# facebookresearch/vilbert-multi-task

Hardware: AMD Instinct MI355X
Metric: samples/sec (36 regions, 36 tokens) ViLBERT-base 6L/6C fwd+bwd (higher is better)
Workload: dtype f32; 1 GPU; bert_base_6layer_6conect.json train_concap step: BertForMultiModalPreTraining fwd+bwd (dropout on) + grad all-reduce + AdamW, 36 regions + 1 global row, batch 256 per GPU, T=36 R=37; per_gpu_batch=256, global_batch=256, parallelism=dp1, visible_gpus=1, launch=eager, gemm_mode=f32, deterministic_wgrad=True, deterministic_fallbacks=0

## Files before the change

### vilbert-multi-task_amd/csrc/attention.hip

```cpp
#include "common.h"
#include "rng.h"

namespace {

#ifdef VB_ATTN_BF16
typedef unsigned short io_t;
__device__ __forceinline__ f32x4 ld4(const io_t* p) {
    const uint2 w = *reinterpret_cast<const uint2*>(p);
    return f32x4{__uint_as_float(w.x << 16), __uint_as_float(w.x & 0xffff0000u), __uint_as_float(w.y << 16),
                 __uint_as_float(w.y & 0xffff0000u)};
}
__device__ __forceinline__ float ld1(const io_t* p) { return __uint_as_float((unsigned)*p << 16); }
__device__ __forceinline__ void st1(io_t* p, float v) { *p = (io_t)vb_bf16_round(v); }
template <int DS>
__device__ __forceinline__ void store_cols(io_t* op, int c, const f32x4 (&a)[DS], int r) {
#pragma unroll
    for (int k = 0; k < DS / 2; ++k) {
        const float even = a[2 * k][r], odd = a[2 * k + 1][r];
        const float recv = __shfl_xor((c & 1) ? even : odd, 1, 64);
        if (c & 1) *reinterpret_cast<unsigned*>(op + 32 * k + 15) = vb_bf16_pack(recv, odd);
        else *reinterpret_cast<unsigned*>(op + 32 * k) = vb_bf16_pack(even, recv);
    }
}
#else
// ... 212 lines not shown
#pragma unroll
                for (int r = 0; r < 4; ++r) st[kt][r] = st[kt][r] * (dp[kt][r] - dsum) * p.scale;
    }

    const io_t* rbase = (BWD ? kbase : vbase) + c;
    const long ldr = BWD ? p.ldk : p.ldv;
    f32x4 oacc[DS];
#pragma unroll
    for (int dt = 0; dt < DS; ++dt) oacc[dt] = f32x4{0.f, 0.f, 0.f, 0.f};
#pragma unroll
    for (int kt = 0; kt < NT; ++kt) {
        if (kt < nkt) {
            f32x4 av, bv[DS];
#pragma unroll
            for (int r = 0; r < 4; ++r) {
                const int key = min(kt * 16 + 4 * g + r, p.n_k - 1);
                const io_t* rp = rbase + (long)key * ldr;
                av[r] = st[kt][r];
#pragma unroll
                for (int dt = 0; dt < DS; ++dt) bv[dt][r] = ld1(rp + 16 * dt);
            }
            mma_rank4<DS>(oacc, av, bv);
        }
    }

    io_t* obase = BWD ? p.dQ : p.O;
    const long ldo = BWD ? p.lddq : p.ldo;
#pragma unroll
    for (int r = 0; r < 4; ++r) {
        const int q = qt * 16 + 4 * g + r;
        if (q < p.n_q) {
            io_t* op = obase + ((long)b * p.n_q + q) * ldo + h * D + c;
            store_cols<DS>(op, c, oacc, r);
        }
    }
}

template <int D>
__global__ __launch_bounds__(256) void attn_bwd_kv_kernel(const AttnP p_in) {
    AttnP p = p_in;
    p.seed = vb_seed_with_epoch(p_in.seed, p_in.epoch);
    const int lane = threadIdx.x & 63;
    const long item = (long)blockIdx.x * 4 + (threadIdx.x >> 6);
    if (item >= p.total) return;
    const int kt = (int)(item % p.n_kt);
    const long bh = item / p.n_kt;
    const int h = (int)(bh % p.heads);
    const int b = (int)(bh / p.heads);
    const int c = lane & 15, g = lane >> 4;
    constexpr int DS = D / 16;
    const bool drop = p.drop_p > 0.f;

    const int key = kt * 16 + c;
    const int k_row = min(key, p.n_k - 1);
    const bool key_ok = key < p.n_k;
    f32x4 kf[DS], vf[DS];
    load_frag<DS>(kf, p.K + ((long)b * p.n_k + k_row) * p.ldk + h * D + 4 * g);
    load_frag<DS>(vf, p.V + ((long)b * p.n_k + k_row) * p.ldv + h * D + 4 * g);
    const float madd = p.mask != nullptr ? p.mask[(long)b * p.n_k + k_row] : 0.f;

    const io_t* qbase = p.Q + (long)b * p.n_q * p.ldq + h * D;
    const io_t* dobase = p.dO + (long)b * p.n_q * p.lddo + h * D;
    const float* lse = p.lse + bh * p.n_q;
    const float* dvec = p.dvec + bh * p.n_q;

    f32x4 dk[DS], dv[DS];
#pragma unroll
    for (int dt = 0; dt < DS; ++dt) {
        dk[dt] = f32x4{0.f, 0.f, 0.f, 0.f};
        dv[dt] = f32x4{0.f, 0.f, 0.f, 0.f};
    }

    for (int qt = 0; qt < p.n_qt; ++qt) {
        const int q_row = min(qt * 16 + c, p.n_q - 1);
        f32x4 qf[DS], dof[DS];
        load_frag<DS>(qf, qbase + (long)q_row * p.ldq + 4 * g);
        load_frag<DS>(dof, dobase + (long)q_row * p.lddo + 4 * g);
        const f32x4 s = dot_tile<DS>(qf, kf);
        const f32x4 dpr = dot_tile<DS>(dof, vf);
        f32x4 pd, dsv;
#pragma unroll
        for (int r = 0; r < 4; ++r) {
            const int q = qt * 16 + 4 * g + r;
            float dsr = 0.f, pdr = 0.f;
            if (q < p.n_q && key_ok) {
                const float sv = __fadd_rn(__fmul_rn(s[r], p.scale), madd);
                const float pv = expf(sv - lse[q]);
                float d = dpr[r];
                pdr = pv;
                if (drop) {
                    const bool keep = vb_keep(p.seed, (uint64_t)((bh * p.n_q + q) * p.n_k + key), p.drop_p);
                    d = keep ? d * p.drop_scale : 0.f;
                    pdr = keep ? pv * p.drop_scale : 0.f;
                }
                dsr = pv * (d - dvec[q]) * p.scale;
            }
            pd[r] = pdr;
            dsv[r] = dsr;
        }
        f32x4 dov[DS], qv[DS];
#pragma unroll
        for (int r = 0; r < 4; ++r) {
            const int q = min(qt * 16 + 4 * g + r, p.n_q - 1);
            const io_t* dop = dobase + (long)q * p.lddo + c;
            const io_t* qp = qbase + (long)q * p.ldq + c;
#pragma unroll
            for (int dt = 0; dt < DS; ++dt) {
                dov[dt][r] = ld1(dop + 16 * dt);
                qv[dt][r] = ld1(qp + 16 * dt);
            }
        }
        mma_rank4<DS>(dv, pd, dov);
        mma_rank4<DS>(dk, dsv, qv);
    }

#pragma unroll
    for (int r = 0; r < 4; ++r) {
        const int kk = kt * 16 + 4 * g + r;
        if (kk < p.n_k) {
            io_t* kp = p.dK + ((long)b * p.n_k + kk) * p.lddk + h * D + c;
            io_t* vp = p.dV + ((long)b * p.n_k + kk) * p.lddv + h * D + c;
            store_cols<DS>(kp, c, dk, r);
            store_cols<DS>(vp, c, dv, r);
        }
    }
}

constexpr int LDS_MAX_ROWS = 48;

template <int D>
__device__ __forceinline__ void stage_rows2(float* __restrict__ s0, const io_t* __restrict__ g0, long ld0,
                                            float* __restrict__ s1, const io_t* __restrict__ g1, long ld1, int n_rows) {
    constexpr int V4 = D / 4, IT = (LDS_MAX_ROWS * V4 + 255) / 256;
    f32x4 r0[IT], r1[IT];
#pragma unroll
    for (int i = 0; i < IT; ++i) {
        const int f = threadIdx.x + 256 * i;
        const int r = min(f / V4, n_rows - 1), c4 = f % V4;
        r0[i] = ld4(g0 + (long)r * ld0 + c4 * 4);
        r1[i] = ld4(g1 + (long)r * ld1 + c4 * 4);
    }
#pragma unroll
    for (int i = 0; i < IT; ++i) {
        const int f = threadIdx.x + 256 * i;
        const int r = f / V4, c4 = f % V4;
        if (f < LDS_MAX_ROWS * V4) {
            const bool real = r < n_rows;
            *reinterpret_cast<f32x4*>(s0 + r * (D + 4) + c4 * 4) = real ? r0[i] : f32x4{0.f, 0.f, 0.f, 0.f};
            *reinterpret_cast<f32x4*>(s1 + r * (D + 4) + c4 * 4) = real ? r1[i] : f32x4{0.f, 0.f, 0.f, 0.f};
        }
    }
}

template <int DS>
__device__ __forceinline__ void load_frag_lds(f32x4 (&f)[DS], const float* s) {
#pragma unroll
    for (int q = 0; q < DS; ++q) f[q] = *reinterpret_cast<const f32x4*>(s + 16 * q);
}

template <int D, bool BWD>
__global__ __launch_bounds__(256, 3) void attn_q_lds_kernel(const AttnP p_in) {
    AttnP p = p_in;
    p.seed = vb_seed_with_epoch(p_in.seed, p_in.epoch);
    extern __shared__ __attribute__((aligned(16))) float smem_att[];
    constexpr int LD = D + 4, DS = D / 16, NT = LDS_MAX_ROWS / 16;
    float* sK = smem_att;
    float* sV = smem_att + LDS_MAX_ROWS * LD;
    const long bh = blockIdx.x;
    const int h = (int)(bh % p.heads), b = (int)(bh / p.heads);
    const int lane = threadIdx.x & 63, wave = threadIdx.x >> 6;
    const int c = lane & 15, g = lane >> 4;
    const int nkt = p.n_kt;
    const bool drop = p.drop_p > 0.f;

    f32x4 qf_first[DS];
    load_frag<DS>(qf_first, p.Q + ((long)b * p.n_q + min(wave * 16 + c, p.n_q - 1)) * p.ldq + h * D + 4 * g);
    stage_rows2<D>(sK, p.K + (long)b * p.n_k * p.ldk + h * D, p.ldk, sV, p.V + (long)b * p.n_k * p.ldv + h * D, p.ldv, p.n_k);
    __syncthreads();
    const float* mrow = p.mask != nullptr ? p.mask + (long)b * p.n_k : nullptr;

    for (int qt = wave; qt < p.n_qt; qt += 4) {
        const int q_row = min(qt * 16 + c, p.n_q - 1);
        f32x4 qf[DS];
        if (qt == wave) {
#pragma unroll
            for (int i = 0; i < DS; ++i) qf[i] = qf_first[i];
        } else {
            load_frag<DS>(qf, p.Q + ((long)b * p.n_q + q_row) * p.ldq + h * D + 4 * g);
        }
        const long prow = (bh * p.n_q + q_row) * p.n_k;

        f32x4 st[NT];
        float mx = -INFINITY;
#pragma unroll
        for (int kt = 0; kt < NT; ++kt) {
            st[kt] = f32x4{-INFINITY, -INFINITY, -INFINITY, -INFINITY};
            if (kt < nkt) {
                f32x4 kf[DS];
                load_frag_lds<DS>(kf, sK + (kt * 16 + c) * LD + 4 * g);
                f32x4 acc = dot_tile<DS>(kf, qf);
#pragma unroll
                for (int r = 0; r < 4; ++r) {
                    const int key = kt * 16 + 4 * g + r;
                    float v = -INFINITY;
                    if (key < p.n_k) {
                        v = __fmul_rn(acc[r], p.scale);
                        if (mrow != nullptr) v = __fadd_rn(v, mrow[key]);
                    }
                    acc[r] = v;
                    mx = fmaxf(mx, v);
                }
                st[kt] = acc;
            }
        }

        if (!BWD) {
            mx = group_max(mx);
            float sum = 0.f;
#pragma unroll
            for (int kt = 0; kt < NT; ++kt)
                if (kt < nkt)
#pragma unroll
                    for (int r = 0; r < 4; ++r) {
                        const float e = expf(st[kt][r] - mx);
                        st[kt][r] = e;
                        sum += e;
                    }
            sum = group_sum(sum);
            const float inv = 1.0f / sum;
            if (p.lse != nullptr && g == 0 && qt * 16 + c < p.n_q) p.lse[bh * p.n_q + qt * 16 + c] = mx + logf(sum);
#pragma unroll
            for (int kt = 0; kt < NT; ++kt)
                if (kt < nkt)
#pragma unroll
                    for (int r = 0; r < 4; ++r) {
                        float pv = st[kt][r] * inv;
                        if (drop) {
                            const int key = kt * 16 + 4 * g + r;
                            pv = vb_keep(p.seed, (uint64_t)(prow + key), p.drop_p) ? pv * p.drop_scale : 0.f;
                        }
                        st[kt][r] = pv;
                    }
            if (p.probs != nullptr && qt * 16 + c < p.n_q) {
                float* pr = p.probs + prow;
#pragma unroll
                for (int kt = 0; kt < NT; ++kt)
                    if (kt < nkt)
#pragma unroll
                        for (int r = 0; r < 4; ++r) {
                            const int key = kt * 16 + 4 * g + r;
                            if (key < p.n_k) pr[key] = st[kt][r];
                        }
            }
        } else {
            const float lse = p.lse[bh * p.n_q + q_row];
            f32x4 dof[DS];
            load_frag<DS>(dof, p.dO + ((long)b * p.n_q + q_row) * p.lddo + h * D + 4 * g);
            f32x4 dp[NT];
            float dsum = 0.f;
#pragma unroll
            for (int kt = 0; kt < NT; ++kt) {
                dp[kt] = f32x4{0.f, 0.f, 0.f, 0.f};
                if (kt < nkt) {
                    f32x4 vf[DS];
                    load_frag_lds<DS>(vf, sV + (kt * 16 + c) * LD + 4 * g);
                    f32x4 acc = dot_tile<DS>(vf, dof);
#pragma unroll
                    for (int r = 0; r < 4; ++r) {
                        const int key = min(kt * 16 + 4 * g + r, p.n_k - 1);
                        const float pv = expf(st[kt][r] - lse);
                        float d = acc[r];
                        if (drop) d = vb_keep(p.seed, (uint64_t)(prow + key), p.drop_p) ? d * p.drop_scale : 0.f;
                        st[kt][r] = pv;
                        acc[r] = d;
                        dsum += pv * d;
                    }
                    dp[kt] = acc;
                }
            }
            dsum = group_sum(dsum);
            if (g == 0 && qt * 16 + c < p.n_q) p.dvec[bh * p.n_q + qt * 16 + c] = dsum;
#pragma unroll
            for (int kt = 0; kt < NT; ++kt)
                if (kt < nkt)
#pragma unroll
                    for (int r = 0; r < 4; ++r) st[kt][r] = st[kt][r] * (dp[kt][r] - dsum) * p.scale;
        }

        const float* rb = (BWD ? sK : sV) + c;
        f32x4 oacc[DS];
#pragma unroll
        for (int dt = 0; dt < DS; ++dt) oacc[dt] = f32x4{0.f, 0.f, 0.f, 0.f};
#pragma unroll
        for (int kt = 0; kt < NT; ++kt) {
            if (kt < nkt) {
                f32x4 av, bv[DS];
#pragma unroll
                for (int r = 0; r < 4; ++r) {
                    const float* rp = rb + (kt * 16 + 4 * g + r) * LD;
                    av[r] = st[kt][r];
#pragma unroll
                    for (int dt = 0; dt < DS; ++dt) bv[dt][r] = rp[16 * dt];
                }
                mma_rank4<DS>(oacc, av, bv);
            }
        }
        io_t* obase = BWD ? p.dQ : p.O;
        const long ldo = BWD ? p.lddq : p.ldo;
#pragma unroll
        for (int r = 0; r < 4; ++r) {
            const int q = qt * 16 + 4 * g + r;
            if (q < p.n_q) {
                io_t* op = obase + ((long)b * p.n_q + q) * ldo + h * D + c;
                store_cols<DS>(op, c, oacc, r);
            }
        }
    }
}

template <int D>
__global__ __launch_bounds__(256) void attn_bwd_kv_lds_kernel(const AttnP p_in) {
    AttnP p = p_in;
    p.seed = vb_seed_with_epoch(p_in.seed, p_in.epoch);
    extern __shared__ __attribute__((aligned(16))) float smem_att[];
    constexpr int LD = D + 4, DS = D / 16;
    float* sQ = smem_att;
    float* sO = smem_att + LDS_MAX_ROWS * LD;
    const long bh = blockIdx.x;
    const int h = (int)(bh % p.heads), b = (int)(bh / p.heads);
    const int lane = threadIdx.x & 63, wave = threadIdx.x >> 6;
    const int c = lane & 15, g = lane >> 4;
    const bool drop = p.drop_p > 0.f;

    stage_rows2<D>(sQ, p.Q + (long)b * p.n_q * p.ldq + h * D, p.ldq, sO, p.dO + (long)b * p.n_q * p.lddo + h * D, p.lddo, p.n_q);
    __syncthreads();
    const float* lse = p.lse + bh * p.n_q;
    const float* dvec = p.dvec + bh * p.n_q;

    for (int kt = wave; kt < p.n_kt; kt += 4) {
        const int key = kt * 16 + c;
        const int k_row = min(key, p.n_k - 1);
        const bool key_ok = key < p.n_k;
        f32x4 kf[DS], vf[DS];
        load_frag<DS>(kf, p.K + ((long)b * p.n_k + k_row) * p.ldk + h * D + 4 * g);
        load_frag<DS>(vf, p.V + ((long)b * p.n_k + k_row) * p.ldv + h * D + 4 * g);
        const float madd = p.mask != nullptr ? p.mask[(long)b * p.n_k + k_row] : 0.f;
        f32x4 dk[DS], dv[DS];
#pragma unroll
        for (int dt = 0; dt < DS; ++dt) {
            dk[dt] = f32x4{0.f, 0.f, 0.f, 0.f};
            dv[dt] = f32x4{0.f, 0.f, 0.f, 0.f};
        }
        for (int qt = 0; qt < p.n_qt; ++qt) {
            f32x4 qf[DS], dof[DS];
            load_frag_lds<DS>(qf, sQ + (qt * 16 + c) * LD + 4 * g);
            load_frag_lds<DS>(dof, sO + (qt * 16 + c) * LD + 4 * g);
            const f32x4 s = dot_tile<DS>(qf, kf);
            const f32x4 dpr = dot_tile<DS>(dof, vf);
            f32x4 pd, dsv;
#pragma unroll
            for (int r = 0; r < 4; ++r) {
                const int q = qt * 16 + 4 * g + r;
                float dsr = 0.f, pdr = 0.f;
                if (q < p.n_q && key_ok) {
                    const float sv = __fadd_rn(__fmul_rn(s[r], p.scale), madd);
                    const float pv = expf(sv - lse[q]);
                    float d = dpr[r];
                    pdr = pv;
                    if (drop) {
                        const bool keep = vb_keep(p.seed, (uint64_t)((bh * p.n_q + q) * p.n_k + key), p.drop_p);
                        d = keep ? d * p.drop_scale : 0.f;
                        pdr = keep ? pv * p.drop_scale : 0.f;
                    }
                    dsr = pv * (d - dvec[q]) * p.scale;
                }
                pd[r] = pdr;
                dsv[r] = dsr;
            }
            f32x4 dov[DS], qv[DS];
#pragma unroll
            for (int r = 0; r < 4; ++r) {
                const float* dop = sO + (qt * 16 + 4 * g + r) * LD + c;
                const float* qp = sQ + (qt * 16 + 4 * g + r) * LD + c;
#pragma unroll
                for (int dt = 0; dt < DS; ++dt) {
                    dov[dt][r] = dop[16 * dt];
                    qv[dt][r] = qp[16 * dt];
                }
            }
            mma_rank4<DS>(dv, pd, dov);
            mma_rank4<DS>(dk, dsv, qv);
        }
#pragma unroll
        for (int r = 0; r < 4; ++r) {
            const int kk = kt * 16 + 4 * g + r;
            if (kk < p.n_k) {
                io_t* kp = p.dK + ((long)b * p.n_k + kk) * p.lddk + h * D + c;
                io_t* vp = p.dV + ((long)b * p.n_k + kk) * p.lddv + h * D + c;
                store_cols<DS>(kp, c, dk, r);
                store_cols<DS>(vp, c, dv, r);
            }
        }
    }
}

template <int D>
__global__ __launch_bounds__(256) void attn_bwd_fused_lds_kernel(const AttnP p_in, const int ps_off) {
    AttnP p = p_in;
    p.seed = vb_seed_with_epoch(p_in.seed, p_in.epoch);
    extern __shared__ __attribute__((aligned(16))) float smem_att[];
    constexpr int LD = D + 4, DS = D / 16, NT = LDS_MAX_ROWS / 16, V4 = D / 4;
    float* sK = smem_att;
    float* sV = sK + p.n_k * LD;
    float* sQ = sV + p.n_k * LD;
    float* sO = sQ + p.n_q * LD;
    float* sD = sO + p.n_q * LD;
    const int LDP = (p.n_k + 3) / 4 * 4 + 4;
    float* sP = smem_att + ps_off;
    float* sS = sP + p.n_q * LDP;
    const long bh = blockIdx.x;
    const int h = (int)(bh % p.heads), b = (int)(bh / p.heads);
    const int lane = threadIdx.x & 63, wave = threadIdx.x >> 6;
    const int c = lane & 15, g = lane >> 4;
    const int nkt = p.n_kt;
    const bool drop = p.drop_p > 0.f;

    {
        const io_t* gk = p.K + (long)b * p.n_k * p.ldk + h * D;
        const io_t* gv = p.V + (long)b * p.n_k * p.ldv + h * D;
        const io_t* gq = p.Q + (long)b * p.n_q * p.ldq + h * D;
        const io_t* go = p.dO + (long)b * p.n_q * p.lddo + h * D;
        constexpr int IT = (LDS_MAX_ROWS * V4 + 255) / 256;
        f32x4 rk[IT], rv[IT], rq[IT], ro[IT];
#pragma unroll
        for (int i = 0; i < IT; ++i) {
            const int f = threadIdx.x + 256 * i;
            const int r = f / V4, c4 = (f % V4) * 4;
            if (r < p.n_k) {
                rk[i] = ld4(gk + (long)r * p.ldk + c4);
                rv[i] = ld4(gv + (long)r * p.ldv + c4);
            }
            if (r < p.n_q) {
                rq[i] = ld4(gq + (long)r * p.ldq + c4);
                ro[i] = ld4(go + (long)r * p.lddo + c4);
            }
        }
#pragma unroll
        for (int i = 0; i < IT; ++i) {
            const int f = threadIdx.x + 256 * i;
            const int r = f / V4, c4 = (f % V4) * 4;
            if (r < p.n_k) {
                *reinterpret_cast<f32x4*>(sK + r * LD + c4) = rk[i];
                *reinterpret_cast<f32x4*>(sV + r * LD + c4) = rv[i];
            }
            if (r < p.n_q) {
                *reinterpret_cast<f32x4*>(sQ + r * LD + c4) = rq[i];
                *reinterpret_cast<f32x4*>(sO + r * LD + c4) = ro[i];
            }
        }
    }
    __syncthreads();
    const float* mrow = p.mask != nullptr ? p.mask + (long)b * p.n_k : nullptr;
    const float* lse_g = p.lse + bh * p.n_q;

    const int qt = wave;
    const bool has_q = qt < p.n_qt;
    f32x4 pdm[NT], dsm[NT];
    if (has_q) {
        const int q_row = min(qt * 16 + c, p.n_q - 1);
        f32x4 qf[DS], dof[DS];
        load_frag_lds<DS>(qf, sQ + q_row * LD + 4 * g);
        load_frag_lds<DS>(dof, sO + q_row * LD + 4 * g);
        const long prow = (bh * p.n_q + q_row) * p.n_k;
        const float lse = lse_g[q_row];
        f32x4 dp[NT];
        float dsum = 0.f;
#pragma unroll
        for (int kt = 0; kt < NT; ++kt) {
            pdm[kt] = f32x4{0.f, 0.f, 0.f, 0.f};
            dsm[kt] = f32x4{0.f, 0.f, 0.f, 0.f};
            dp[kt] = f32x4{0.f, 0.f, 0.f, 0.f};
            if (kt < nkt) {
                const int krow = min(kt * 16 + c, p.n_k - 1);
                f32x4 kf[DS], vf[DS];
                load_frag_lds<DS>(kf, sK + krow * LD + 4 * g);
                load_frag_lds<DS>(vf, sV + krow * LD + 4 * g);
                const f32x4 sacc = dot_tile<DS>(kf, qf);
                f32x4 dacc = dot_tile<DS>(vf, dof);
#pragma unroll
                for (int r = 0; r < 4; ++r) {
                    const int key = kt * 16 + 4 * g + r;
                    float pv = 0.f, d = 0.f, pd = 0.f;
                    if (key < p.n_k) {
                        float sv = __fmul_rn(sacc[r], p.scale);
                        if (mrow != nullptr) sv = __fadd_rn(sv, mrow[key]);
                        pv = expf(sv - lse);
                        d = dacc[r];
                        pd = pv;
                        if (drop) {
                            const bool keep = vb_keep(p.seed, (uint64_t)(prow + key), p.drop_p);
                            d = keep ? d * p.drop_scale : 0.f;
                            pd = keep ? pv * p.drop_scale : 0.f;
                        }
                    }
                    dsm[kt][r] = pv;
                    pdm[kt][r] = pd;
                    dacc[r] = d;
                    dsum += pv * d;
                }
                dp[kt] = dacc;
            }
        }
        dsum = group_sum(dsum);
#pragma unroll
        for (int kt = 0; kt < NT; ++kt)
            if (kt < nkt)
#pragma unroll
                for (int r = 0; r < 4; ++r) dsm[kt][r] = dsm[kt][r] * (dp[kt][r] - dsum) * p.scale;
        f32x4 oacc[DS];
#pragma unroll
        for (int dt = 0; dt < DS; ++dt) oacc[dt] = f32x4{0.f, 0.f, 0.f, 0.f};
#pragma unroll
        for (int kt = 0; kt < NT; ++kt) {
            if (kt < nkt) {
                f32x4 av, bv[DS];
#pragma unroll
                for (int r = 0; r < 4; ++r) {
                    const float* rp = sK + min(kt * 16 + 4 * g + r, p.n_k - 1) * LD + c;
                    av[r] = dsm[kt][r];
#pragma unroll
                    for (int dt = 0; dt < DS; ++dt) bv[dt][r] = rp[16 * dt];
                }
                mma_rank4<DS>(oacc, av, bv);
            }
        }
#pragma unroll
        for (int r = 0; r < 4; ++r) {
            const int q = qt * 16 + 4 * g + r;
            if (q < p.n_q) {
                io_t* op = p.dQ + ((long)b * p.n_q + q) * p.lddq + h * D + c;
                store_cols<DS>(op, c, oacc, r);
            }
        }
    }
    __syncthreads();
    if (has_q && qt * 16 + c < p.n_q) {
        float* pr = sP + (qt * 16 + c) * LDP + 4 * g;
        float* sr = sS + (qt * 16 + c) * LDP + 4 * g;
#pragma unroll
        for (int kt = 0; kt < NT; ++kt)
            if (kt < nkt && kt * 16 + 4 * g < LDP) {
                *reinterpret_cast<f32x4*>(pr + kt * 16) = pdm[kt];
                *reinterpret_cast<f32x4*>(sr + kt * 16) = dsm[kt];
            }
    }
    __syncthreads();

    for (int kt = wave; kt < p.n_kt; kt += 4) {
        const int key = min(kt * 16 + c, p.n_k - 1);
        f32x4 dk[DS], dv[DS];
#pragma unroll
        for (int dt = 0; dt < DS; ++dt) {
            dk[dt] = f32x4{0.f, 0.f, 0.f, 0.f};
            dv[dt] = f32x4{0.f, 0.f, 0.f, 0.f};
        }
        for (int q4 = 0; q4 < p.n_q; q4 += 16) {
            f32x4 pd, dsv, dov[DS], qv[DS];
#pragma unroll
            for (int r = 0; r < 4; ++r) {
                const int q = q4 + 4 * g + r;
                const int qr = min(q, p.n_q - 1);
                pd[r] = q < p.n_q ? sP[qr * LDP + key] : 0.f;
                dsv[r] = q < p.n_q ? sS[qr * LDP + key] : 0.f;
                const float* dop = sO + qr * LD + c;
                const float* qp = sQ + qr * LD + c;
#pragma unroll
                for (int dt = 0; dt < DS; ++dt) {
                    dov[dt][r] = dop[16 * dt];
                    qv[dt][r] = qp[16 * dt];
                }
            }
            mma_rank4<DS>(dv, pd, dov);
            mma_rank4<DS>(dk, dsv, qv);
        }
#pragma unroll
        for (int r = 0; r < 4; ++r) {
            const int kk = kt * 16 + 4 * g + r;
            if (kk < p.n_k) {
                io_t* kp = p.dK + ((long)b * p.n_k + kk) * p.lddk + h * D + c;
                io_t* vp = p.dV + ((long)b * p.n_k + kk) * p.lddv + h * D + c;
                store_cols<DS>(kp, c, dk, r);
                store_cols<DS>(vp, c, dv, r);
            }
        }
    }
}

template <int D>
int launch_bwd_fused_lds(hipStream_t st, const AttnP& p) {
    const int ldp = (p.n_k + 3) / 4 * 4 + 4;
    const int base = (2 * p.n_k + 2 * p.n_q) * (D + 4) + LDS_MAX_ROWS;
    const bool over_v = 2 * p.n_q * ldp <= p.n_k * (D + 4);
    const int ps_off = over_v ? p.n_k * (D + 4) : base;
    const int bytes = (over_v ? base : base + 2 * p.n_q * ldp) * 4;
    static const hipError_t attr = hipFuncSetAttribute(reinterpret_cast<const void*>(&attn_bwd_fused_lds_kernel<D>),
                                                       hipFuncAttributeMaxDynamicSharedMemorySize, 160 * 1024);
    if (attr != hipSuccess) return (int)attr;
    hipLaunchKernelGGL((attn_bwd_fused_lds_kernel<D>), dim3((unsigned)(p.batch * p.heads)), dim3(256), bytes, st, p, ps_off);
    VB_LAUNCH_CHECK();
    return 0;
}

inline bool use_lds_path(const AttnP& p) {
    static const int on = vb_env_int("VB_ATTN_LDS", 1);
    return on && p.n_q <= LDS_MAX_ROWS && p.n_k <= LDS_MAX_ROWS && p.q_bstride == p.n_q && p.kv_bstride == p.n_k;
}

template <int D, bool BWD>
int launch_q_lds(hipStream_t st, const AttnP& p) {
    constexpr int bytes = 2 * LDS_MAX_ROWS * (D + 4) * 4;
    hipLaunchKernelGGL((attn_q_lds_kernel<D, BWD>), dim3((unsigned)(p.batch * p.heads)), dim3(256), bytes, st, p);
    VB_LAUNCH_CHECK();
    return 0;
}

template <int D>
int launch_kv_lds(hipStream_t st, const AttnP& p) {
    constexpr int bytes = 2 * LDS_MAX_ROWS * (D + 4) * 4;
    hipLaunchKernelGGL((attn_bwd_kv_lds_kernel<D>), dim3((unsigned)(p.batch * p.heads)), dim3(256), bytes, st, p);
    VB_LAUNCH_CHECK();
    return 0;
}

template <int D, bool BWD>
int launch_q(hipStream_t st, const AttnP& p) {
    if (use_lds_path(p) && p.dvec_mode == VB_DVEC_COMPUTE) return launch_q_lds<D, BWD>(st, p);
    dim3 block(256), grid((unsigned)((p.total + 3) / 4));
    if (p.n_kt <= 3) hipLaunchKernelGGL((attn_q_kernel<D, 3, BWD>), grid, block, 0, st, p);
    else if (p.n_kt <= 8) hipLaunchKernelGGL((attn_q_kernel<D, 8, BWD>), grid, block, 0, st, p);
    else if (p.n_kt <= 20) hipLaunchKernelGGL((attn_q_kernel<D, 20, BWD>), grid, block, 0, st, p);
    else return VB_E_RANGE;
    VB_LAUNCH_CHECK();
    return 0;
}

template <int D>
int launch_kv(hipStream_t st, const AttnP& p) {
    if (use_lds_path(p)) return launch_kv_lds<D>(st, p);
    dim3 block(256), grid((unsigned)((p.total + 3) / 4));
    hipLaunchKernelGGL((attn_bwd_kv_kernel<D>), grid, block, 0, st, p);
    VB_LAUNCH_CHECK();
    return 0;
}

#ifdef VB_ATTN_BF16
typedef vb_attention_bf16_args attn_args_t;
typedef vb_attention_bf16_grads attn_grads_t;
#define VB_ATTN_FWD vb_attention_fwd_bf16
#define VB_ATTN_BWD vb_attention_bwd_bf16
constexpr unsigned IO_ALIGN = 7u;
#else
typedef vb_attention_args attn_args_t;
typedef vb_attention_grads attn_grads_t;
#define VB_ATTN_FWD vb_attention_fwd
#define VB_ATTN_BWD vb_attention_bwd
constexpr unsigned IO_ALIGN = 15u;
#endif
inline bool io_aligned(const void* q) { return (reinterpret_cast<uintptr_t>(q) & IO_ALIGN) == 0; }

int fill_common(AttnP& p, const attn_args_t* a) {
    if (a == nullptr || a->Q == nullptr || a->K == nullptr || a->V == nullptr) return VB_E_BADARG;
    if (a->batch <= 0 || a->heads <= 0 || a->n_q <= 0 || a->n_k <= 0) return VB_E_BADARG;
    if (a->n_k > VB_MAX_KEYS) return VB_E_RANGE;
    if ((a->q_batch != a->batch && a->q_batch != 1) || (a->kv_batch != a->batch && a->kv_batch != 1))
        return VB_E_BADARG;
    if (!(a->dropout_p >= 0.f && a->dropout_p < 1.f)) return VB_E_BADARG;
    if ((a->ldq | a->ldk | a->ldv) % 4 != 0 || !io_aligned(a->Q) || !io_aligned(a->K) || !io_aligned(a->V))
        return VB_E_ALIGN;
    p.batch = a->batch; p.heads = a->heads; p.n_q = a->n_q; p.n_k = a->n_k;
    p.n_qt = (a->n_q + 15) / 16;
    p.n_kt = (a->n_k + 15) / 16;
    p.q_bstride = a->q_batch == 1 && a->batch > 1 ? 0 : a->n_q;
    p.kv_bstride = a->kv_batch == 1 && a->batch > 1 ? 0 : a->n_k;
    p.m_bstride = p.kv_bstride;
    p.Q = a->Q; p.ldq = a->ldq; p.K = a->K; p.ldk = a->ldk; p.V = a->V; p.ldv = a->ldv;
    p.mask = a->mask_add; p.scale = a->scale; p.lse = a->lse;
    p.drop_p = a->dropout_p; p.drop_scale = 1.0f / (1.0f - a->dropout_p); p.seed = a->seed;
    p.epoch = a->dropout_p > 0.f ? vb_seed_epoch() : nullptr;
    return 0;
}

}

extern "C" int VB_ATTN_FWD(void* stream, const attn_args_t* a) {
    AttnP p{};
    if (int e = fill_common(p, a)) return e;
    if (a->O == nullptr) return VB_E_BADARG;
    p.O = a->O; p.ldo = a->ldo; p.probs = a->probs;
    p.total = (long)a->batch * a->heads * p.n_qt;
    hipStream_t st = static_cast<hipStream_t>(stream);
    switch (a->head_dim) {
        case 32: return launch_q<32, false>(st, p);
        case 64: return launch_q<64, false>(st, p);
        case 128: return launch_q<128, false>(st, p);
        default: return VB_E_RANGE;
    }
}

extern "C" int VB_ATTN_BWD(void* stream, const attn_args_t* a, const attn_grads_t* gr) {
    AttnP p{};
    if (int e = fill_common(p, a)) return e;
    if (gr == nullptr || gr->dO == nullptr || gr->dQ == nullptr || gr->dK == nullptr || gr->dV == nullptr ||
        gr->dvec == nullptr || a->lse == nullptr)
        return VB_E_BADARG;
    if (a->q_batch != a->batch || a->kv_batch != a->batch) return VB_E_BADARG;
    if (gr->lddo % 4 != 0 || !io_aligned(gr->dO)) return VB_E_ALIGN;
    p.dO = gr->dO; p.lddo = gr->lddo;
    p.dQ = gr->dQ; p.lddq = gr->lddq; p.dK = gr->dK; p.lddk = gr->lddk; p.dV = gr->dV; p.lddv = gr->lddv;
    p.dvec = gr->dvec;
    p.dvec_mode = gr->dvec_mode;
    if (p.dvec_mode < VB_DVEC_COMPUTE || p.dvec_mode > VB_DVEC_GIVEN) return VB_E_BADARG;
    hipStream_t st = static_cast<hipStream_t>(stream);
    int e = 0;
    static const int fused = vb_env_int("VB_ATTN_FUSED_BWD", 1);
    if (p.dvec_mode == VB_DVEC_COMPUTE && fused && use_lds_path(p) && (gr->lddq | gr->lddk | gr->lddv) % 4 == 0) {
        switch (a->head_dim) {
            case 32: return launch_bwd_fused_lds<32>(st, p);
            case 64: return launch_bwd_fused_lds<64>(st, p);
            case 128: return launch_bwd_fused_lds<128>(st, p);
            default: return VB_E_RANGE;
        }
    }
    p.total = (long)a->batch * a->heads * p.n_qt;
    switch (a->head_dim) {
        case 32: e = launch_q<32, true>(st, p); break;
        case 64: e = launch_q<64, true>(st, p); break;
        case 128: e = launch_q<128, true>(st, p); break;
        default: return VB_E_RANGE;
    }
    if (e) return e;
    if (p.dvec_mode == VB_DVEC_ACCUMULATE) return 0;
    p.total = (long)a->batch * a->heads * p.n_kt;
    switch (a->head_dim) {
        case 32: return launch_kv<32>(st, p);
        case 64: return launch_kv<64>(st, p);
        default: return launch_kv<128>(st, p);
    }
}
```

### vilbert-multi-task_amd/csrc/layernorm.hip

```cpp
#include "rowops.h"
#include "rng.h"

using namespace vbrow;

namespace {

template <int NV>
__global__ __launch_bounds__(256) void layernorm_kernel(long rows, int n_cols, const float* __restrict__ x,
                                                        const float* __restrict__ x2,
                                                        const float* __restrict__ gamma,
                                                        const float* __restrict__ beta, float eps,
                                                        float* __restrict__ y, float* mean, float* rstd,
                                                        unsigned char* __restrict__ q, long ldq,
                                                        float* __restrict__ qscale, unsigned* __restrict__ mxs,
                                                        long mxs_rows) {
    const int lane = threadIdx.x & 63;
    const long row = (long)blockIdx.x * ROWS_PER_BLOCK + (threadIdx.x >> 6);
    if (row >= rows) return;
    const float* xr = x + row * n_cols;
    f32x4 v[NV];
#pragma unroll
    for (int i = 0; i < NV; ++i) {
        const int col = VB_LANE_COL(i, lane);
        v[i] = f32x4{0.f, 0.f, 0.f, 0.f};
// ... 148 lines not shown
    f32x4 gam[NV], dg[NV], db[NV];
#pragma unroll
    for (int i = 0; i < NV; ++i) {
        const int col = VB_LANE_COL(i, lane);
        gam[i] = col < n_cols ? *reinterpret_cast<const f32x4*>(gamma + col) : f32x4{0.f, 0.f, 0.f, 0.f};
        dg[i] = f32x4{0.f, 0.f, 0.f, 0.f};
        db[i] = f32x4{0.f, 0.f, 0.f, 0.f};
    }
    [[maybe_unused]] typename IO::packed ndy[NV], nx[NV];
    [[maybe_unused]] float nmu = 0.f, nrs = 0.f;
    [[maybe_unused]] auto fetch = [&](long row) {
#pragma unroll
        for (int i = 0; i < NV; ++i) {
            const int col = VB_LANE_COL(i, lane);
            ndy[i] = IO::zero();
            nx[i] = IO::zero();
            if (col < n_cols) {
                ndy[i] = *reinterpret_cast<const typename IO::packed*>(dy + row * n_cols + col);
                nx[i] = *reinterpret_cast<const typename IO::packed*>(x + row * n_cols + col);
            }
        }
        nmu = mean[row];
        nrs = rstd[row];
    };
    if constexpr (IO::PREFETCH)
        if (row_begin < rows) fetch(row_begin);
    for (int rr = 0; rr < LNB_ROWS_PER_WAVE; ++rr) {
        const long row = row_begin + rr;
        if (row >= rows) break;
        const float mu = IO::PREFETCH ? nmu : mean[row], rs = IO::PREFETCH ? nrs : rstd[row];
        f32x4 xh[NV], g[NV];
        [[maybe_unused]] f32x4 dcur[NV];
        if constexpr (IO::PREFETCH) {
#pragma unroll
            for (int i = 0; i < NV; ++i) {
                dcur[i] = IO::unpack(ndy[i]);
                xh[i] = IO::unpack(nx[i]);
            }
            if (rr + 1 < LNB_ROWS_PER_WAVE && row + 1 < rows) fetch(row + 1);
        }
        float s1 = 0.f, s2 = 0.f;
#pragma unroll
        for (int i = 0; i < NV; ++i) {
            const int col = VB_LANE_COL(i, lane);
            if constexpr (!IO::PREFETCH) xh[i] = f32x4{0.f, 0.f, 0.f, 0.f};
            g[i] = f32x4{0.f, 0.f, 0.f, 0.f};
            if (col < n_cols) {
                const f32x4 d = IO::PREFETCH ? dcur[i] : *reinterpret_cast<const f32x4*>(dy + row * n_cols + col);
                xh[i] = ((IO::PREFETCH ? xh[i] : *reinterpret_cast<const f32x4*>(x + row * n_cols + col)) - mu) * rs;
                g[i] = d * gam[i];
                dg[i] += d * xh[i];
                db[i] += d;
                s1 += (g[i][0] + g[i][1]) + (g[i][2] + g[i][3]);
                s2 += (g[i][0] * xh[i][0] + g[i][1] * xh[i][1]) + (g[i][2] * xh[i][2] + g[i][3] * xh[i][3]);
            }
        }
        const float m1 = wave_sum(s1) / (float)n_cols, m2 = wave_sum(s2) / (float)n_cols;
#pragma unroll
        for (int i = 0; i < NV; ++i) {
            const int col = VB_LANE_COL(i, lane);
            if (col < n_cols) {
                const f32x4 d = (g[i] - m1 - xh[i] * m2) * rs;
                IO::store(dx + row * n_cols + col, d);
                if (dxd != nullptr) {
                    f32x4 dd;
                    const uint64_t idx = (uint64_t)(row * n_cols + col);
#pragma unroll
                    for (int e = 0; e < 4; ++e) dd[e] = vb_keep(seed, idx + e, drop_p) ? d[e] * drop_scale : 0.f;
                    IO::store(dxd + row * n_cols + col, dd);
                }
            }
        }
    }
    constexpr bool BLOCK_REDUCE = NV <= 4;
    __shared__ f32x4 red[BLOCK_REDUCE ? 3 * 2 * NV * 64 : 1];
    if (BLOCK_REDUCE) {
        if (wave > 0) {
#pragma unroll
            for (int i = 0; i < NV; ++i) {
                red[((wave - 1) * 2 * NV + i) * 64 + lane] = dg[i];
                red[((wave - 1) * 2 * NV + NV + i) * 64 + lane] = db[i];
            }
        }
        __syncthreads();
        if (wave > 0) return;
#pragma unroll
        for (int w2 = 0; w2 < 3; ++w2)
#pragma unroll
            for (int i = 0; i < NV; ++i) {
                dg[i] += red[(w2 * 2 * NV + i) * 64 + lane];
                db[i] += red[(w2 * 2 * NV + NV + i) * 64 + lane];
            }
    }
    float* w = ws + (BLOCK_REDUCE ? (long)blockIdx.x : part) * 2 * n_cols;
#pragma unroll
    for (int i = 0; i < NV; ++i) {
        const int col = VB_LANE_COL(i, lane);
        if (col < n_cols) {
            *reinterpret_cast<f32x4*>(w + col) = dg[i];
            *reinterpret_cast<f32x4*>(w + n_cols + col) = db[i];
        }
    }
}

__global__ __launch_bounds__(256) void layernorm_bwd_wide_kernel(long rows, int n_cols, const float* __restrict__ dy,
                                                                 const float* __restrict__ x,
                                                                 const float* __restrict__ mean,
                                                                 const float* __restrict__ rstd,
                                                                 const float* __restrict__ gamma,
                                                                 float* __restrict__ dx, float* __restrict__ ws) {
    const int lane = threadIdx.x & 63;
    const long row = (long)blockIdx.x * 4 + (threadIdx.x >> 6);
    if (row >= rows) return;
    const float mu = mean[row], rs = rstd[row];
    const float* __restrict__ dyr = dy + row * n_cols;
    const float* __restrict__ xr = x + row * n_cols;
    float s1 = 0.f, s2 = 0.f;
    for (int col = lane * 4; col < n_cols; col += 256) {
        const f32x4 d = *reinterpret_cast<const f32x4*>(dyr + col);
        const f32x4 xh = (*reinterpret_cast<const f32x4*>(xr + col) - mu) * rs;
        const f32x4 g = d * *reinterpret_cast<const f32x4*>(gamma + col);
        s1 += (g[0] + g[1]) + (g[2] + g[3]);
        s2 += (g[0] * xh[0] + g[1] * xh[1]) + (g[2] * xh[2] + g[3] * xh[3]);
    }
    const float m1 = wave_sum(s1) / (float)n_cols, m2 = wave_sum(s2) / (float)n_cols;
    float* __restrict__ w = ws + row * 2 * n_cols;
    for (int col = lane * 4; col < n_cols; col += 256) {
        const f32x4 d = *reinterpret_cast<const f32x4*>(dyr + col);
        const f32x4 xh = (*reinterpret_cast<const f32x4*>(xr + col) - mu) * rs;
        const f32x4 g = d * *reinterpret_cast<const f32x4*>(gamma + col);
        *reinterpret_cast<f32x4*>(dx + row * n_cols + col) = (g - m1 - xh * m2) * rs;
        *reinterpret_cast<f32x4*>(w + col) = d * xh;
        *reinterpret_cast<f32x4*>(w + n_cols + col) = d;
    }
}

template <int INFLIGHT>
__global__ __launch_bounds__(1024) void colreduce_kernel(long parts, int width, const float* __restrict__ ws,
                                                         float* __restrict__ out0, float* __restrict__ out1, int n_cols) {
    static_assert(INFLIGHT == 1 || INFLIGHT == 4, "instantiated forms");
    __shared__ float red[16][INFLIGHT == 1 ? 64 : 65];
    const int c = threadIdx.x & 63, pg = threadIdx.x >> 6;
    const int col = blockIdx.x * 64 + c;
    float s0 = 0.f, s1 = 0.f, s2 = 0.f, s3 = 0.f;
    if (col < width) {
        long p = pg;
        if constexpr (INFLIGHT == 4)
            for (; p + 48 < parts; p += 64) {
                s0 += ws[p * width + col];
                s1 += ws[(p + 16) * width + col];
                s2 += ws[(p + 32) * width + col];
                s3 += ws[(p + 48) * width + col];
            }
        for (; p < parts; p += 16) s0 += ws[p * width + col];
    }
    red[pg][c] = INFLIGHT == 4 ? (s0 + s1) + (s2 + s3) : s0;
    __syncthreads();
    if (pg == 0 && col < width) {
        float t = 0.f;
#pragma unroll
        for (int i = 0; i < 16; ++i) t += red[i][c];
        if (col < n_cols) out0[col] = t;
        else out1[col - n_cols] = t;
    }
}

template <int INFLIGHT>
int launch_colreduce(hipStream_t st, long parts, int n_cols, const float* ws, float* dgamma, float* dbeta) {
    const int width = 2 * n_cols;
    hipLaunchKernelGGL(colreduce_kernel<INFLIGHT>, dim3((unsigned)((width + 63) / 64)), dim3(1024), 0, st, parts, width, ws,
                       dgamma, dbeta, n_cols);
    VB_LAUNCH_CHECK();
    return 0;
}

inline bool codes_ok(const void* q, int64_t ldq, int n_cols) { return ldq >= n_cols && ldq % 4 == 0 && all_aligned(4, {q}); }

int launch_layernorm(void* stream, int64_t rows, int32_t n_cols, const float* x, const float* x2, const float* gamma,
                     const float* beta, float eps, float* y, float* mean, float* rstd, uint8_t* q, int64_t ldq,
                     float* qscale, uint32_t* mxs, int64_t mxs_rows) {
    if (!all_aligned(16, {x, x2, y, gamma, beta}) || (q != nullptr && !codes_ok(q, ldq, n_cols)) || !all_aligned(4, {mxs}))
        return VB_E_ALIGN;
    const dim3 grid((unsigned)((rows + ROWS_PER_BLOCK - 1) / ROWS_PER_BLOCK)), block(256);
    dispatch_nv<32>(nv_for(n_cols), [&](auto nv) {
        hipLaunchKernelGGL((layernorm_kernel<decltype(nv)::value>), grid, block, 0, static_cast<hipStream_t>(stream), (long)rows,
                           n_cols, x, x2, gamma, beta, eps, y, mean, rstd, q, (long)ldq, qscale, mxs, (long)mxs_rows);
    });
    VB_LAUNCH_CHECK();
    return 0;
}

template <int R, int MAX, typename Emit>
void launch_layernorm16(void* stream, int64_t rows, int32_t n_cols, const uint16_t* x, const float* gamma, const float* beta,
                        float eps, uint16_t* y, const Emit out) {
    const dim3 grid((unsigned)((rows + R * ROWS_PER_BLOCK - 1) / (R * ROWS_PER_BLOCK))), block(256);
    dispatch_nv<MAX>(nv_for(n_cols), [&](auto nv) {
        hipLaunchKernelGGL((layernorm16_kernel<decltype(nv)::value, R, Emit>), grid, block, 0, static_cast<hipStream_t>(stream),
                           (long)rows, n_cols, x, gamma, beta, eps, y, out);
    });
}

template <typename IO, int MAX, int INFLIGHT>
int layernorm_bwd_impl(void* stream, int64_t rows, int32_t n_cols, const typename IO::elem* dy, const typename IO::elem* x,
                       const float* mean, const float* rstd, const float* gamma, typename IO::elem* dx, float* dgamma,
                       float* dbeta, float* workspace, typename IO::elem* dxd, float drop_p, uint64_t seed) {
    if (!all_aligned(IO::ALIGN, {dy, x, dx, dxd}) || !all_aligned(16, {gamma, workspace})) return VB_E_ALIGN;
    hipStream_t st = static_cast<hipStream_t>(stream);
    const long blocks = lnb_blocks(rows);
    const float dscale = dxd != nullptr ? 1.0f / (1.0f - drop_p) : 1.0f;
    const uint64_t* epoch = vb_seed_epoch();
    dispatch_nv<MAX>(nv_for(n_cols), [&](auto nv) {
        hipLaunchKernelGGL((layernorm_bwd_kernel<decltype(nv)::value, IO>), dim3((unsigned)blocks), dim3(256), 0, st, (long)rows,
                           n_cols, dy, x, mean, rstd, gamma, dx, workspace, dxd, drop_p, dscale, seed, epoch);
    });
    VB_LAUNCH_CHECK();
    return launch_colreduce<INFLIGHT>(st, nv_for(n_cols) <= 4 ? blocks : blocks * 4, n_cols, workspace, dgamma, dbeta);
}

int layernorm_bwd_f32(void* stream, int64_t rows, int32_t n_cols, const float* dy, const float* x, const float* mean,
                      const float* rstd, const float* gamma, float* dx, float* dgamma, float* dbeta, float* workspace,
                      float* dxd, float drop_p, uint64_t seed) {
    if (any_null({dy, x, mean, rstd, gamma, dx, dgamma, dbeta, workspace}) || rows <= 0) return VB_E_BADARG;
    if (int e = check_cols(n_cols)) return e;
    if (nv_for(n_cols) <= 16)
        return layernorm_bwd_impl<RowF32, 16, 1>(stream, rows, n_cols, dy, x, mean, rstd, gamma, dx, dgamma, dbeta, workspace,
                                                 dxd, drop_p, seed);
    if (!all_aligned(16, {dy, x, dx, gamma, workspace})) return VB_E_ALIGN;
    if (dxd != nullptr) return VB_E_RANGE;
    hipStream_t st = static_cast<hipStream_t>(stream);
    hipLaunchKernelGGL(layernorm_bwd_wide_kernel, dim3((unsigned)((rows + 3) / 4)), dim3(256), 0, st, (long)rows, n_cols, dy, x,
                       mean, rstd, gamma, dx, workspace);
    VB_LAUNCH_CHECK();
    return launch_colreduce<1>(st, rows, n_cols, workspace, dgamma, dbeta);
}

}

extern "C" int vb_layernorm_fwd(void* stream, int64_t rows, int32_t n_cols, const float* x, const float* x2,
                                const float* gamma, const float* beta, float eps, float* y, float* mean,
                                float* rstd) {
    if (any_null({x, gamma, beta, y}) || rows <= 0) return VB_E_BADARG;
    if (int e = check_cols(n_cols)) return e;
    return launch_layernorm(stream, rows, n_cols, x, x2, gamma, beta, eps, y, mean, rstd, nullptr, 0, nullptr, nullptr, 0);
}

extern "C" int vb_layernorm_fwd_fp8(void* stream, int64_t rows, int32_t n_cols, const float* x, const float* x2,
                                    const float* gamma, const float* beta, float eps, float* y, uint8_t* q,
                                    int64_t ldq, float* qscale) {
    if (any_null({x, gamma, beta, y, q, qscale}) || rows <= 0) return VB_E_BADARG;
    if (int e = check_cols(n_cols)) return e;
    return launch_layernorm(stream, rows, n_cols, x, x2, gamma, beta, eps, y, nullptr, nullptr, q, ldq, qscale, nullptr, 0);
}

extern "C" int vb_layernorm_fwd_mx(void* stream, int64_t rows, int32_t n_cols, const float* x, const float* x2,
                                   const float* gamma, const float* beta, float eps, float* y, uint8_t* q, int64_t ldq,
                                   uint32_t* scales, int64_t scale_rows) {
    if (any_null({x, gamma, beta, y, q, scales}) || rows <= 0) return VB_E_BADARG;
    if (int e = check_cols(n_cols)) return e;
    if (n_cols % 128 != 0 || scale_rows < rows) return VB_E_RANGE;
    return launch_layernorm(stream, rows, n_cols, x, x2, gamma, beta, eps, y, nullptr, nullptr, q, ldq, nullptr, scales,
                            scale_rows);
}

extern "C" int vb_layernorm_fwd_mx16(void* stream, int64_t rows, int32_t n_cols, const uint16_t* x, const float* gamma,
                                     const float* beta, float eps, uint16_t* y, uint8_t* q, int64_t ldq, uint32_t* scales,
                                     int64_t scale_rows) {
    if (any_null({x, gamma, beta, y, q, scales}) || rows <= 0) return VB_E_BADARG;
    if (int e = check_cols(n_cols)) return e;
    if (n_cols % 128 != 0 || scale_rows < rows) return VB_E_RANGE;
    if (!all_aligned(RowBF16::ALIGN, {x, y}) || !all_aligned(16, {gamma, beta}) || !codes_ok(q, ldq, n_cols) ||
        !all_aligned(4, {scales}))
        return VB_E_ALIGN;
    const EmitMX out{q, (long)ldq, scales, (long)scale_rows};
    if ((rows + 2 * ROWS_PER_BLOCK - 1) / (2 * ROWS_PER_BLOCK) <= 2048 || n_cols > 1024)
        launch_layernorm16<2, 32>(stream, rows, n_cols, x, gamma, beta, eps, y, out);
    else
        launch_layernorm16<4, 4>(stream, rows, n_cols, x, gamma, beta, eps, y, out);
    VB_LAUNCH_CHECK();
    return 0;
}

extern "C" int vb_layernorm_fwd_bf16(void* stream, int64_t rows, int32_t n_cols, const uint16_t* x, const float* gamma,
                                     const float* beta, float eps, uint16_t* y, float* mean, float* rstd) {
    if (any_null({x, gamma, beta, y}) || rows <= 0) return VB_E_BADARG;
    if (n_cols <= 0 || n_cols % 4 != 0 || n_cols > 1024) return VB_E_RANGE;
    if (!all_aligned(RowBF16::ALIGN, {x, y}) || !all_aligned(16, {gamma, beta})) return VB_E_ALIGN;
    const EmitStats out{mean, rstd};
    if (rows < 4096) launch_layernorm16<1, 4>(stream, rows, n_cols, x, gamma, beta, eps, y, out);
    else if ((rows + 7) / 8 <= 2048) launch_layernorm16<2, 4>(stream, rows, n_cols, x, gamma, beta, eps, y, out);
    else launch_layernorm16<4, 4>(stream, rows, n_cols, x, gamma, beta, eps, y, out);
    VB_LAUNCH_CHECK();
    return 0;
}

extern "C" int64_t vb_layernorm_bwd_workspace(int64_t rows, int32_t n_cols) {
    if (rows <= 0 || n_cols <= 0) return 0;
    if (nv_for(n_cols) > 16) return rows * 2 * n_cols;
    const int64_t parts = (rows + LNB_ROWS_PER_WAVE - 1) / LNB_ROWS_PER_WAVE;
    const int64_t parts_padded = (parts + 3) / 4 * 4;
    return parts_padded * 2 * n_cols;
}

extern "C" int vb_layernorm_bwd(void* stream, int64_t rows, int32_t n_cols, const float* dy, const float* x,
                                const float* mean, const float* rstd, const float* gamma, float* dx,
                                float* dgamma, float* dbeta, float* workspace) {
    return layernorm_bwd_f32(stream, rows, n_cols, dy, x, mean, rstd, gamma, dx, dgamma, dbeta, workspace, nullptr, 0.f, 0);
// ... 26 lines not shown
```

Baseline: 2590 samples/s.

## Shrink fused attention-backward LDS footprint and batch colreduce loads

The fused attention backward kernel now stages only K and V into shared memory at first. Q and dO fragments are loaded straight from global into registers, and the full Q/dO tiles are loaded into registers early and written to LDS later, reusing the K/V region once scores are done. This lowers dynamic LDS per block, and launch bounds now ask for 3 or 4 blocks per CU so more blocks can run at once. Scores against all key tiles are precomputed before the dV loop. The deterministic colreduce (INFLIGHT=1) path issues 16 loads ahead per iteration while keeping summation order. This adds register pressure and longer live ranges.

After: 2599 samples/s (median of 6 runs). No clear change (+0.3%).

```diff
diff --git a/vilbert-multi-task_amd/csrc/attention.hip b/vilbert-multi-task_amd/csrc/attention.hip
--- a/vilbert-multi-task_amd/csrc/attention.hip
+++ b/vilbert-multi-task_amd/csrc/attention.hip
@@ -388,6 +388,29 @@
     }
 }
 
+template <int D>
+__device__ __forceinline__ void stage_rows2_exact(float* __restrict__ s0, const io_t* __restrict__ g0, long ld0,
+                                                  float* __restrict__ s1, const io_t* __restrict__ g1, long ld1, int n_rows) {
+    constexpr int V4 = D / 4, IT = (LDS_MAX_ROWS * V4 + 255) / 256;
+    f32x4 r0[IT], r1[IT];
+#pragma unroll
+    for (int i = 0; i < IT; ++i) {
+        const int f = threadIdx.x + 256 * i;
+        const int r = min(f / V4, n_rows - 1), c4 = (f % V4) * 4;
+        r0[i] = ld4(g0 + (long)r * ld0 + c4);
+        r1[i] = ld4(g1 + (long)r * ld1 + c4);
+    }
+#pragma unroll
+    for (int i = 0; i < IT; ++i) {
+        const int f = threadIdx.x + 256 * i;
+        const int r = f / V4, c4 = (f % V4) * 4;
+        if (r < n_rows) {
+            *reinterpret_cast<f32x4*>(s0 + r * (D + 4) + c4) = r0[i];
+            *reinterpret_cast<f32x4*>(s1 + r * (D + 4) + c4) = r1[i];
+        }
+    }
+}
+
 template <int DS>
 __device__ __forceinline__ void load_frag_lds(f32x4 (&f)[DS], const float* s) {
 #pragma unroll
@@ -641,16 +664,18 @@
 }
 
 template <int D>
-__global__ __launch_bounds__(256) void attn_bwd_fused_lds_kernel(const AttnP p_in, const int ps_off) {
+constexpr int bwd_fused_blocks_per_cu() { return D >= 128 ? 3 : 4; }
+
+template <int D>
+__global__ __launch_bounds__(256, bwd_fused_blocks_per_cu<D>()) void attn_bwd_fused_lds_kernel(const AttnP p_in, const int ps_off) {
     AttnP p = p_in;
     p.seed = vb_seed_with_epoch(p_in.seed, p_in.epoch);
     extern __shared__ __attribute__((aligned(16))) float smem_att[];
     constexpr int LD = D + 4, DS = D / 16, NT = LDS_MAX_ROWS / 16, V4 = D / 4;
     float* sK = smem_att;
     float* sV = sK + p.n_k * LD;
-    float* sQ = sV + p.n_k * LD;
+    float* sQ = smem_att;
     float* sO = sQ + p.n_q * LD;
-    float* sD = sO + p.n_q * LD;
     const int LDP = (p.n_k + 3) / 4 * 4 + 4;
     float* sP = smem_att + ps_off;
     float* sS = sP + p.n_q * LDP;
@@ -661,54 +686,44 @@
     const int nkt = p.n_kt;
     const bool drop = p.drop_p > 0.f;
 
+    const io_t* gq = p.Q + (long)b * p.n_q * p.ldq + h * D;
+    const io_t* go = p.dO + (long)b * p.n_q * p.lddo + h * D;
+    const int qt = wave;
+    const bool has_q = qt < p.n_qt;
+    f32x4 qf[DS], dof[DS];
     {
-        const io_t* gk = p.K + (long)b * p.n_k * p.ldk + h * D;
-        const io_t* gv = p.V + (long)b * p.n_k * p.ldv + h * D;
-        const io_t* gq = p.Q + (long)b * p.n_q * p.ldq + h * D;
-        const io_t* go = p.dO + (long)b * p.n_q * p.lddo + h * D;
-        constexpr int IT = (LDS_MAX_ROWS * V4 + 255) / 256;
-        f32x4 rk[IT], rv[IT], rq[IT], ro[IT];
-#pragma unroll
-        for (int i = 0; i < IT; ++i) {
-            const int f = threadIdx.x + 256 * i;
-            const int r = f / V4, c4 = (f % V4) * 4;
-            if (r < p.n_k) {
-                rk[i] = ld4(gk + (long)r * p.ldk + c4);
-                rv[i] = ld4(gv + (long)r * p.ldv + c4);
-            }
-            if (r < p.n_q) {
-                rq[i] = ld4(gq + (long)r * p.ldq + c4);
-                ro[i] = ld4(go + (long)r * p.lddo + c4);
-            }
-        }
-#pragma unroll
-        for (int i = 0; i < IT; ++i) {
-            const int f = threadIdx.x + 256 * i;
-            const int r = f / V4, c4 = (f % V4) * 4;
-            if (r < p.n_k) {
-                *reinterpret_cast<f32x4*>(sK + r * LD + c4) = rk[i];
-                *reinterpret_cast<f32x4*>(sV + r * LD + c4) = rv[i];
-            }
-            if (r < p.n_q) {
-                *reinterpret_cast<f32x4*>(sQ + r * LD + c4) = rq[i];
-                *reinterpret_cast<f32x4*>(sO + r * LD + c4) = ro[i];
-            }
-        }
-    }
+        const int q_row = min(qt * 16 + c, p.n_q - 1);
+        load_frag<DS>(qf, gq + (long)q_row * p.ldq + 4 * g);
+        load_frag<DS>(dof, go + (long)q_row * p.lddo + 4 * g);
+    }
+    stage_rows2_exact<D>(sK, p.K + (long)b * p.n_k * p.ldk + h * D, p.ldk, sV, p.V + (long)b * p.n_k * p.ldv + h * D, p.ldv,
+                         p.n_k);
     __syncthreads();
+    constexpr int IT = (LDS_MAX_ROWS * V4 + 255) / 256;
+    f32x4 rq[IT], ro[IT];
+#pragma unroll
+    for (int i = 0; i < IT; ++i) {
+        const int f = threadIdx.x + 256 * i;
+        const int r = min(f / V4, p.n_q - 1), c4 = (f % V4) * 4;
+        rq[i] = ld4(gq + (long)r * p.ldq + c4);
+        ro[i] = ld4(go + (long)r * p.lddo + c4);
+    }
     const float* mrow = p.mask != nullptr ? p.mask + (long)b * p.n_k : nullptr;
     const float* lse_g = p.lse + bh * p.n_q;
 
-    const int qt = wave;
-    const bool has_q = qt < p.n_qt;
     f32x4 pdm[NT], dsm[NT];
     if (has_q) {
         const int q_row = min(qt * 16 + c, p.n_q - 1);
-        f32x4 qf[DS], dof[DS];
-        load_frag_lds<DS>(qf, sQ + q_row * LD + 4 * g);
-        load_frag_lds<DS>(dof, sO + q_row * LD + 4 * g);
         const long prow = (bh * p.n_q + q_row) * p.n_k;
         const float lse = lse_g[q_row];
+        f32x4 sc[NT];
+#pragma unroll
+        for (int kt = 0; kt < NT; ++kt)
+            if (kt < nkt) {
+                f32x4 kf[DS];
+                load_frag_lds<DS>(kf, sK + min(kt * 16 + c, p.n_k - 1) * LD + 4 * g);
+                sc[kt] = dot_tile<DS>(kf, qf);
+            }
         f32x4 dp[NT];
         float dsum = 0.f;
 #pragma unroll
@@ -718,10 +733,9 @@
             dp[kt] = f32x4{0.f, 0.f, 0.f, 0.f};
             if (kt < nkt) {
                 const int krow = min(kt * 16 + c, p.n_k - 1);
-                f32x4 kf[DS], vf[DS];
-                load_frag_lds<DS>(kf, sK + krow * LD + 4 * g);
+                f32x4 vf[DS];
                 load_frag_lds<DS>(vf, sV + krow * LD + 4 * g);
-                const f32x4 sacc = dot_tile<DS>(kf, qf);
+                const f32x4 sacc = sc[kt];
                 f32x4 dacc = dot_tile<DS>(vf, dof);
 #pragma unroll
                 for (int r = 0; r < 4; ++r) {
@@ -780,6 +794,15 @@
         }
     }
     __syncthreads();
+#pragma unroll
+    for (int i = 0; i < IT; ++i) {
+        const int f = threadIdx.x + 256 * i;
+        const int r = f / V4, c4 = (f % V4) * 4;
+        if (r < p.n_q) {
+            *reinterpret_cast<f32x4*>(sQ + r * LD + c4) = rq[i];
+            *reinterpret_cast<f32x4*>(sO + r * LD + c4) = ro[i];
+        }
+    }
     if (has_q && qt * 16 + c < p.n_q) {
         float* pr = sP + (qt * 16 + c) * LDP + 4 * g;
         float* sr = sS + (qt * 16 + c) * LDP + 4 * g;
@@ -835,10 +858,9 @@
 template <int D>
 int launch_bwd_fused_lds(hipStream_t st, const AttnP& p) {
     const int ldp = (p.n_k + 3) / 4 * 4 + 4;
-    const int base = (2 * p.n_k + 2 * p.n_q) * (D + 4) + LDS_MAX_ROWS;
-    const bool over_v = 2 * p.n_q * ldp <= p.n_k * (D + 4);
-    const int ps_off = over_v ? p.n_k * (D + 4) : base;
-    const int bytes = (over_v ? base : base + 2 * p.n_q * ldp) * 4;
+    const int ps_off = 2 * p.n_q * (D + 4);
+    const int kv = 2 * p.n_k * (D + 4), qo = ps_off + 2 * p.n_q * ldp;
+    const int bytes = (kv > qo ? kv : qo) * 4;
     static const hipError_t attr = hipFuncSetAttribute(reinterpret_cast<const void*>(&attn_bwd_fused_lds_kernel<D>),
                                                        hipFuncAttributeMaxDynamicSharedMemorySize, 160 * 1024);
     if (attr != hipSuccess) return (int)attr;
diff --git a/vilbert-multi-task_amd/csrc/layernorm.hip b/vilbert-multi-task_amd/csrc/layernorm.hip
--- a/vilbert-multi-task_amd/csrc/layernorm.hip
+++ b/vilbert-multi-task_amd/csrc/layernorm.hip
@@ -324,6 +324,17 @@
                 s2 += ws[(p + 32) * width + col];
                 s3 += ws[(p + 48) * width + col];
             }
+        if constexpr (INFLIGHT == 1) {
+            constexpr int AHEAD = 16;
+            for (; p < parts; p += 16 * AHEAD) {
+                float v[AHEAD];
+#pragma unroll
+                for (int i = 0; i < AHEAD; ++i) v[i] = p + 16 * i < parts ? ws[(p + 16 * i) * width + col] : 0.f;
+#pragma unroll
+                for (int i = 0; i < AHEAD; ++i)
+                    if (p + 16 * i < parts) s0 += v[i];
+            }
+        }
         for (; p < parts; p += 16) s0 += ws[p * width + col];
     }
     red[pg][c] = INFLIGHT == 4 ? (s0 + s1) + (s2 + s3) : s0;
```
